# GabeTsai/YOLO-For-Turbines

Measured on AMD Instinct MI355X. Metric: images/sec at 416x416 (fwd), higher is better.
Workload: dtype f32; 1 GPU; BASELINE configs[1]: batch 32/GPU 416x416 fp32 inference, 80-class head, YOLOv3 forward (75 fused conv launches); per_gpu_batch=32, global_batch=32, image_size=416, num_classes=80, parallelism=image-sharded x1 (no collective)

## Files before the change

include/yolo_mi355x.h:

```cpp
#ifndef YOLO_MI355X_H
#define YOLO_MI355X_H

#include <stddef.h>
#include <stdint.h>

#ifdef __cplusplus
extern "C" {
#endif

#define YOLO_OK 0
#define YOLO_ERR_ARG (-1)
#define YOLO_ERR_UNSUPPORTED (-2)
#define YOLO_ERR_LAUNCH (-3)
#define YOLO_ERR_WORKSPACE (-4)

enum { YOLO_F32 = 0, YOLO_F16 = 1, YOLO_BF16 = 2 };
enum { YOLO_ACT_NONE = 0, YOLO_ACT_LEAKY = 1, YOLO_ACT_MISH = 2 };
enum { YOLO_OUT_NHWC = 0, YOLO_OUT_UPSAMPLE2X = 1, YOLO_OUT_HEAD = 2 };
enum { YOLO_FLAG_RESIDUAL = 1, YOLO_FLAG_NANCHECK = 2, YOLO_FLAG_FILTERS_READY = 4, YOLO_FLAG_SPLIT_BF16 = 8 };

typedef struct yolo_conv_desc {
    int32_t n, h, w;
    int32_t cin, cout;
    int32_t ksize, stride;
    int32_t x_ld, x_off;
    int32_t y_ld, y_off;
    int32_t r_ld, r_off;
    int32_t act;
    int32_t out_mode;
    int32_t dtype;
    int32_t flags;
    int32_t tile;
} yolo_conv_desc;

// ... 23 lines not shown
int yolo_stem_supported(int cin, int cout, int ksize, int stride);
int yolo_stem_pack(const float* w_oihw, float* w_k_major, int cout, void* stream);
int yolo_stem_fwd(const float* x_nchw, const float* w_k_major, const float* scale, const float* shift, void* y,
                  int n, int h, int w, int cout, int y_ld, int y_off, int act, int dtype, int32_t* nan_flag, void* stream);

int yolo_conv_fwd(const yolo_conv_desc* d, const void* x, const void* w_packed, const float* scale,
                  const float* shift, const void* residual, void* y, int32_t* nan_flag, void* stream);
int yolo_conv_fwd_batch(const yolo_conv_op* ops, int n_ops, int32_t* nan_flag, void* stream);
size_t yolo_conv_workspace_bytes(const yolo_conv_desc* d);
int yolo_conv_fwd_ws(const yolo_conv_desc* d, const void* x, const void* w_packed, const float* scale, const float* shift,
                     const void* residual, void* y, void* workspace, size_t workspace_bytes, int32_t* nan_flag, void* stream);
int yolo_conv_pick_tile(const yolo_conv_desc* d);
int yolo_conv_num_tiles(void);
int yolo_conv_split3_supported(const yolo_conv_desc* d);
int yolo_conv_split3_eligible(const yolo_conv_desc* d);
size_t yolo_wino4_filter_bytes(const yolo_conv_desc* d);
int yolo_wino4_filters(const yolo_conv_desc* d, const void* w_packed, void* U4, void* stream);
int yolo_conv_wino4_blocks(const yolo_conv_desc* d, int* whole, int* half);

size_t yolo_bn_workspace_bytes(int m, int c);
int yolo_bn_stats(const void* z, int m, int c, int ld, int off, const float* gamma, const float* beta, float momentum,
                  float eps, float* running_mean, float* running_var, float* mean, float* invstd, float* scale,
                  float* shift, int dtype, void* workspace, size_t workspace_bytes, void* stream);
int yolo_conv_stats_rows(const yolo_conv_desc* d, int* ld);
int yolo_conv_fwd_stats(const yolo_conv_desc* d, const void* x, const void* w_packed, void* z, float* stats, size_t stats_bytes,
                        void* stream);
int yolo_bn_stats_from_partials(const float* partial, int rows, int ld, int m, int c, const float* gamma, const float* beta,
                                float momentum, float eps, float* running_mean, float* running_var, float* mean, float* invstd,
                                float* scale, float* shift, void* stream);
int yolo_conv_bstats_rows(const yolo_conv_desc* d, int* ld);
// ... 127 lines not shown
```

yolo_for_turbines_amd/_lib.py:

```python
from __future__ import annotations

import ctypes as C
import os

_HERE = os.path.dirname(os.path.abspath(__file__))
LIB_PATH = os.environ.get("YOLO_MI355X_LIB") or os.path.join(_HERE, "libyolo_mi355x.so")

F32, F16, BF16 = 0, 1, 2
ACT_NONE, ACT_LEAKY, ACT_MISH = 0, 1, 2
OUT_NHWC, OUT_UPSAMPLE2X, OUT_HEAD = 0, 1, 2
FLAG_RESIDUAL, FLAG_NANCHECK, FLAG_FILTERS_READY, FLAG_SPLIT_BF16 = 1, 2, 4, 8


class PackItem(C.Structure):
    _fields_ = [("w_oihw", C.c_void_p), ("w_packed", C.c_void_p), ("cout", C.c_int), ("cin", C.c_int), ("ksize", C.c_int),
                ("reserved", C.c_int)]


class ConvDesc(C.Structure):
    _fields_ = [(n, C.c_int32) for n in (
        "n", "h", "w", "cin", "cout", "ksize", "stride", "x_ld", "x_off", "y_ld", "y_off", "r_ld", "r_off",
        "act", "out_mode", "dtype", "flags", "tile")]


class ConvOp(C.Structure):
    _fields_ = [("d", ConvDesc)] + [(n, C.c_uint64) for n in ("x", "w_packed", "scale", "shift", "residual", "y",
# ... 48 lines not shown
    "yolo_sgd_step_amp": (C.c_int, [C.c_void_p, C.c_int, C.c_void_p, C.c_int, C.c_void_p, C.c_void_p, C.c_void_p, C.c_void_p, C.c_int, C.c_int,
                                    C.c_void_p]),
    "yolo_stem_supported": (C.c_int, [C.c_int, C.c_int, C.c_int, C.c_int]),
    "yolo_stem_pack": (C.c_int, [C.c_void_p, C.c_void_p, C.c_int, C.c_void_p]),
    "yolo_stem_fwd": (C.c_int, [C.c_void_p, C.c_void_p, C.c_void_p, C.c_void_p, C.c_void_p, C.c_int, C.c_int, C.c_int,
                                C.c_int, C.c_int, C.c_int, C.c_int, C.c_int, C.c_void_p, C.c_void_p]),
    "yolo_conv_fwd": (C.c_int, [C.POINTER(ConvDesc), C.c_void_p, C.c_void_p, C.c_void_p, C.c_void_p, C.c_void_p,
                                C.c_void_p, C.c_void_p, C.c_void_p]),
    "yolo_conv_fwd_batch": (C.c_int, [C.POINTER(ConvOp), C.c_int, C.c_void_p, C.c_void_p]),
    "yolo_conv_workspace_bytes": (C.c_size_t, [C.POINTER(ConvDesc)]),
    "yolo_conv_fwd_ws": (C.c_int, [C.POINTER(ConvDesc), C.c_void_p, C.c_void_p, C.c_void_p, C.c_void_p, C.c_void_p,
                                   C.c_void_p, C.c_void_p, C.c_size_t, C.c_void_p, C.c_void_p]),
    "yolo_conv_pick_tile": (C.c_int, [C.POINTER(ConvDesc)]),
    "yolo_conv_split3_eligible": (C.c_int, [C.POINTER(ConvDesc)]),
    "yolo_conv_split3_supported": (C.c_int, [C.POINTER(ConvDesc)]),
    "yolo_conv_num_tiles": (C.c_int, []),
    "yolo_wino4_filter_bytes": (C.c_size_t, [C.POINTER(ConvDesc)]),
    "yolo_wino4_filters": (C.c_int, [C.POINTER(ConvDesc), C.c_void_p, C.c_void_p, C.c_void_p]),
    "yolo_conv_wino4_blocks": (C.c_int, [C.POINTER(ConvDesc), C.POINTER(C.c_int), C.POINTER(C.c_int)]),
    "yolo_bn_workspace_bytes": (C.c_size_t, [C.c_int, C.c_int]),
    "yolo_bn_stats": (C.c_int, [C.c_void_p, C.c_int, C.c_int, C.c_int, C.c_int, C.c_void_p, C.c_void_p, C.c_float, C.c_float,
                                C.c_void_p, C.c_void_p, C.c_void_p, C.c_void_p, C.c_void_p, C.c_void_p, C.c_int, C.c_void_p,
                                C.c_size_t, C.c_void_p]),
    "yolo_conv_stats_rows": (C.c_int, [C.POINTER(ConvDesc), C.POINTER(C.c_int)]),
    "yolo_conv_fwd_stats": (C.c_int, [C.POINTER(ConvDesc), C.c_void_p, C.c_void_p, C.c_void_p, C.c_void_p, C.c_size_t, C.c_void_p]),
    "yolo_bn_stats_from_partials": (C.c_int, [C.c_void_p, C.c_int, C.c_int, C.c_int, C.c_int, C.c_void_p, C.c_void_p, C.c_float, C.c_float,
                                              C.c_void_p, C.c_void_p, C.c_void_p, C.c_void_p, C.c_void_p, C.c_void_p, C.c_void_p]),
    "yolo_bn_act_fwd": (C.c_int, [C.c_void_p, C.c_int, C.c_int, C.c_void_p, C.c_void_p, C.c_void_p, C.c_void_p, C.c_int, C.c_int,
                                  C.c_void_p, C.c_int, C.c_int, C.c_int, C.c_int, C.c_int, C.c_int, C.c_int, C.c_int, C.c_int,
                                  C.c_void_p, C.c_void_p]),
# ... 108 lines not shown
```

yolo_for_turbines_amd/csrc/conv_f32.hip:

```cpp
#include "conv_f32_epilogue.h"

namespace yolo {

constexpr int LDS_LD = 36;


template <int BM, int BN, bool SMALLC>
__global__ __launch_bounds__(256) void conv_igemm_f32(const ConvArgs p) {
    constexpr int WM = BM / 2, WN = BN / 2;
    constexpr int TM = WM / 32, TN = WN / 32;
    constexpr int RA = BM / 32, RB = BN / 32;
    extern __shared__ __attribute__((aligned(16))) char smem_raw[];
    float* As = reinterpret_cast<float*>(smem_raw);
    float* Bs = As + 2 * BM * LDS_LD;

    const int tid = threadIdx.x;
    const int lane = tid & 63;
    const int wave = tid >> 6;
    const int wm = wave >> 1, wn = wave & 1;
    const int tile_n = blockIdx.x % p.tiles_n;
    const int tile_m = blockIdx.x / p.tiles_n;
    const int m0 = tile_m * BM, n0 = tile_n * BN;

    const int chunk = tid & 7;
// ... 165 lines not shown

static int conv_fwd_impl(const yolo_conv_desc* d, const void* x, const void* w, const float* scale, const float* shift,
                         const void* residual, void* y, void* ws, size_t ws_bytes, int32_t* nan_flag, hipStream_t s) {
    int rc = validate(d);
    if (rc) return rc;
    if (!x || !w || !scale || !shift || !y) return fail(YOLO_ERR_ARG, "conv: null pointer");
    if ((d->flags & YOLO_FLAG_RESIDUAL) && !residual) return fail(YOLO_ERR_ARG, "conv: residual flag without pointer");
    if ((d->flags & YOLO_FLAG_NANCHECK) && !nan_flag) return fail(YOLO_ERR_ARG, "conv: nancheck flag without pointer");
    const bool filters_ready = d->flags & YOLO_FLAG_FILTERS_READY;
    if (filters_ready && (d->dtype != YOLO_F32 || f32_family(d, residual, ws ? ws_bytes : 0) != F32Family::Wino4))
        return fail(YOLO_ERR_ARG, "conv: YOLO_FLAG_FILTERS_READY on a layer that does not run as Winograd F(4x4) (tile 15 with its workspace)");
    const bool split3 = d->flags & YOLO_FLAG_SPLIT_BF16;
    if (split3 && !split3_honoured(d, residual, ws ? ws_bytes : 0))
        return fail(YOLO_ERR_UNSUPPORTED, "conv: YOLO_FLAG_SPLIT_BF16 needs an fp32 layer of the direct kernels (no Winograd workspace in play) with "
                                          "ksize 1 or 3, stride 1 or 2 and cin %% 32 == 0");
    if (d->dtype != YOLO_F32) return conv_h16_launch(d, x, w, scale, shift, residual, y, nan_flag, s);
    ConvArgs a;
    a.x = (const float*)x; a.w = (const float*)w; a.scale = scale; a.shift = shift;
    a.res = (const float*)residual; a.y = (float*)y; a.nan_flag = nan_flag;
    a.N = d->n; a.H = d->h; a.W = d->w; a.Cin = cin_pad_of(d->cin); a.Cout = d->cout;
    a.ks = d->ksize; a.stride = d->stride; a.pad = d->ksize / 2;
    a.Ho = (d->h + 2 * a.pad - d->ksize) / d->stride + 1;
    a.Wo = (d->w + 2 * a.pad - d->ksize) / d->stride + 1;
    const long long M = (long long)d->n * a.Ho * a.Wo;
    if (M > 0x7fffffffLL) return fail(YOLO_ERR_UNSUPPORTED, "conv: N*Ho*Wo exceeds int32");
    a.M = (int)M;
    a.x_ld = d->x_ld; a.x_off = d->x_off; a.y_ld = d->y_ld; a.y_off = d->y_off; a.r_ld = d->r_ld; a.r_off = d->r_off;
    a.Kpad = kpad_of(d->cin, d->ksize);
    a.KT = a.Kpad / BK;
    a.act = d->act; a.out_mode = d->out_mode; a.flags = d->flags;
    a.nc5 = d->out_mode == YOLO_OUT_HEAD ? d->cout / 3 : 1;
    a.tiles_n = 0;
    const bool smallc = a.Cin == 4;
    if (split3) return conv_split3_launch(a, d->tile == kTileF32Rs ? 0 : d->tile, s);
    switch (f32_family(d, residual, ws ? ws_bytes : 0)) {
    case F32Family::Rs: return conv1_rs_launch(d, x, w, scale, shift, residual, y, nan_flag, s);
    case F32Family::Wino4:
        if (!wino4_supported(d)) return fail(YOLO_ERR_UNSUPPORTED, "conv: tile 15 needs fp32 3x3 stride 1 with NHWC output and channel counts %% 4 == 0");
        return conv_wino4_launch(d, x, filters_ready ? nullptr : (const float*)w, filters_ready ? (const float*)w : nullptr, scale, shift,
                                 residual, y, ws, ws_bytes, nan_flag, s);
    case F32Family::Wino: {
        if (!wino_supported(d)) return fail(YOLO_ERR_UNSUPPORTED, "conv: tile 13 needs fp32 3x3 stride 1 with NHWC output and channel counts %% 4 == 0");
        const float* U = (const float*)w + v0_packed_elems(d->cout, d->cin, d->ksize) + v2_frag_elems(d->cout, d->cin, d->ksize);
        return conv_wino_launch(d, x, U, scale, shift, residual, y, ws, ws_bytes, nan_flag, s);
    }
    case F32Family::Direct: break;
    }
    if (d->tile == kTileF32Rs) return fail(YOLO_ERR_UNSUPPORTED, "conv: tile 12 needs a 1x1 with 256 / 384 / 512 input channels and cout %% 128 == 0");
    const int t = d->tile ? d->tile : pick_direct_tile(d);
// ... 20 lines not shown
int yolo_conv_pick_tile(const yolo_conv_desc* d) {
    int rc = yolo::validate(d);
    if (rc) return rc;
    return yolo::pick_tile(d);
}

int yolo_conv_split3_supported(const yolo_conv_desc* d) {
    if (yolo::validate(d)) return 0;
    yolo_conv_desc h = *d;
    h.tile = 0;
    return yolo::split3_honoured(&h, nullptr, SIZE_MAX);
}

int yolo_conv_split3_eligible(const yolo_conv_desc* d) { return yolo_conv_split3_supported(d) && yolo::split3_eligible(d); }

int yolo_conv_fwd(const yolo_conv_desc* d, const void* x, const void* w_packed, const float* scale, const float* shift,
                  const void* residual, void* y, int32_t* nan_flag, void* stream) {
    return yolo::conv_fwd_impl(d, x, w_packed, scale, shift, residual, y, nullptr, 0, nan_flag, (hipStream_t)stream);
}

size_t yolo_conv_workspace_bytes(const yolo_conv_desc* d) {
    if (yolo::validate(d)) return 0;
    switch (yolo::f32_family(d, nullptr, SIZE_MAX)) {
    case yolo::F32Family::Wino4: return yolo::wino4_workspace_bytes(d);
    case yolo::F32Family::Wino: return yolo::wino_workspace_bytes(d);
    default: return 0;
    }
}

int yolo_conv_fwd_ws(const yolo_conv_desc* d, const void* x, const void* w_packed, const float* scale, const float* shift,
// ... 18 lines not shown
```

yolo_for_turbines_amd/csrc/conv_f32_epilogue.h:

```cpp
#pragma once
#include "common.h"

namespace yolo {

typedef float f32x16 __attribute__((ext_vector_type(16)));

struct ConvArgs {
    const float* x;
    const float* w;
    const float* scale;
    const float* shift;
    const float* res;
    float* y;
    int* nan_flag;
    int N, H, W, Cin, Cout, Ho, Wo, M;
    int ks, stride, pad;
    int x_ld, x_off, y_ld, y_off, r_ld, r_off;
    int Kpad, KT;
    int act, out_mode, flags;
    int nc5;
    int tiles_n;
};

constexpr int BK = 32;

bool split3_supported(const yolo_conv_desc* d);
bool split3_eligible(const yolo_conv_desc* d);
int conv_split3_launch(const ConvArgs& a, int tile, hipStream_t s);

template <int BM, int BN>
__device__ __forceinline__ void conv_f32_epilogue(const ConvArgs& p, f32x16 (&acc)[BM / 64][BN / 64], float* ost, int m0, int n0) {
    constexpr int WM = BM / 2, WN = BN / 2;
    constexpr int TM = WM / 32, TN = WN / 32;
    const int tid = threadIdx.x;
    const int lane = tid & 63;
    const int wave = tid >> 6;
    const int wm = wave >> 1, wn = wave & 1;
    const int frow = lane & 31, fh = lane >> 5;
    const int HoWo = p.Ho * p.Wo;
    const bool has_res = p.flags & YOLO_FLAG_RESIDUAL;
    const bool nan_chk = p.flags & YOLO_FLAG_NANCHECK;
    bool saw_nan = false;
    const bool aligned4 = ((p.y_ld | p.y_off) & 3) == 0 && (!has_res || ((p.r_ld | p.r_off) & 3) == 0);
// ... 93 lines not shown
```

yolo_for_turbines_amd/csrc/conv_split3_f32.hip:

```cpp
#include "conv_f32_epilogue.h"

namespace yolo {

typedef __bf16 s3_bf16x8 __attribute__((ext_vector_type(8)));
typedef unsigned int s3_u32x4 __attribute__((ext_vector_type(4)));

constexpr int S3_ROWB = 64;

__device__ __forceinline__ unsigned s3_pack(unsigned a, unsigned b) { return __builtin_amdgcn_perm(b, a, 0x07060302u); }

__device__ __forceinline__ void s3_split(const f32x4 v, u32x2& hi, u32x2& mid, u32x2& lo, f32x4& chk) {
    const s3_u32x4 vb = __builtin_bit_cast(s3_u32x4, v);
    const f32x4 h = __builtin_bit_cast(f32x4, vb & 0xffff0000u);
    const f32x4 r1 = v - h;
    const s3_u32x4 r1b = __builtin_bit_cast(s3_u32x4, r1);
    const f32x4 m = __builtin_bit_cast(f32x4, r1b & 0xffff0000u);
    const f32x4 r2 = r1 - m;
    const s3_u32x4 r2b = __builtin_bit_cast(s3_u32x4, r2);
    chk += r2 * 0.f;
    hi[0] = s3_pack(vb[0], vb[1]); hi[1] = s3_pack(vb[2], vb[3]);
    mid[0] = s3_pack(r1b[0], r1b[1]); mid[1] = s3_pack(r1b[2], r1b[3]);
    lo[0] = s3_pack(r2b[0], r2b[1]); lo[1] = s3_pack(r2b[2], r2b[3]);
}

template <int BM, int BN>
__global__ __launch_bounds__(256, 2) void conv_split3_f32(const ConvArgs p) {
    constexpr int WM = BM / 2, WN = BN / 2;
    constexpr int TM = WM / 32, TN = WN / 32;
    constexpr int RA = BM / 32, RB = BN / 32;
    constexpr bool DBUF = BM + BN <= 128;
    constexpr int A_BYTES = 3 * BM * S3_ROWB;
    constexpr int BUF_BYTES = 3 * (BM + BN) * S3_ROWB;
    extern __shared__ __attribute__((aligned(16))) char smem_raw[];

    const int tid = threadIdx.x;
    const int lane = tid & 63;
    const int wave = tid >> 6;
    const int wm = wave >> 1, wn = wave & 1;
    const int tile_n = blockIdx.x % p.tiles_n;
    const int tile_m = blockIdx.x / p.tiles_n;
    const int m0 = tile_m * BM, n0 = tile_n * BN;
    const int HoWo = p.Ho * p.Wo;

    auto row_geom = [&](int m, long long& base, unsigned& mask) {
        const bool mv = m < p.M;
        const int mm = mv ? m : 0;
        const int n = mm / HoWo;
// ... 5 lines not shown
        unsigned mk = 0;
        for (int kh = 0; kh < p.ks; ++kh)
            for (int kw = 0; kw < p.ks; ++kw)
                if (mv && (unsigned)(hi0 + kh) < (unsigned)p.H && (unsigned)(wi0 + kw) < (unsigned)p.W)
                    mk |= 1u << (kh * p.ks + kw);
        mask = mk;
    };

    const int chunk = tid & 7;
    const int lrow = tid >> 3;
    long long a_base[RA];
    unsigned a_mask[RA];
#pragma unroll
    for (int i = 0; i < RA; ++i) row_geom(m0 + lrow + 32 * i, a_base[i], a_mask[i]);
    const float* wrow = p.w + (size_t)(n0 + lrow) * p.Kpad + chunk * 4;

    f32x4 ra[RA], rb[RB];
    f32x4 chk = {0.f, 0.f, 0.f, 0.f};
    auto load_global = [&](int kt) {
        const int kg = kt * BK;
        const int tap = kg / p.Cin;
        const int coff = kg - tap * p.Cin + chunk * 4;
        const int kh = tap / p.ks, kw = tap - kh * p.ks;
        const long long toff = (long long)(kh * p.W + kw) * p.x_ld + coff;
#pragma unroll
        for (int i = 0; i < RA; ++i) {
            const bool v = (a_mask[i] >> tap) & 1u;
            f32x4 z = {0.f, 0.f, 0.f, 0.f};
            ra[i] = v ? *reinterpret_cast<const f32x4*>(p.x + a_base[i] + toff) : z;
        }
#pragma unroll
        for (int i = 0; i < RB; ++i)
            rb[i] = *reinterpret_cast<const f32x4*>(wrow + (size_t)(32 * i) * p.Kpad + kt * BK);
    };
    auto store_lds = [&](int buf) {
        char* a = smem_raw + buf * BUF_BYTES + lrow * S3_ROWB + (((chunk >> 1) ^ ((lrow >> 2) & 3)) * 16 + (chunk & 1) * 8);
        char* b = a + A_BYTES;
#pragma unroll
        for (int i = 0; i < RA; ++i) {
            u32x2 h, m, l;
            s3_split(ra[i], h, m, l, chk);
            *reinterpret_cast<u32x2*>(a + (0 * BM + 32 * i) * S3_ROWB) = h;
            *reinterpret_cast<u32x2*>(a + (1 * BM + 32 * i) * S3_ROWB) = m;
            *reinterpret_cast<u32x2*>(a + (2 * BM + 32 * i) * S3_ROWB) = l;
        }
#pragma unroll
        for (int i = 0; i < RB; ++i) {
            u32x2 h, m, l;
            s3_split(rb[i], h, m, l, chk);
            *reinterpret_cast<u32x2*>(b + (0 * BN + 32 * i) * S3_ROWB) = h;
            *reinterpret_cast<u32x2*>(b + (1 * BN + 32 * i) * S3_ROWB) = m;
            *reinterpret_cast<u32x2*>(b + (2 * BN + 32 * i) * S3_ROWB) = l;
        }
    };

    f32x16 acc[TM][TN];
#pragma unroll
    for (int i = 0; i < TM; ++i)
#pragma unroll
        for (int j = 0; j < TN; ++j)
#pragma unroll
            for (int r = 0; r < 16; ++r) acc[i][j][r] = 0.f;

    const int frow = lane & 31, fh = lane >> 5;
    const int a_frag = (wm * WM + frow) * S3_ROWB;
    const int b_frag = A_BYTES + (wn * WN + frow) * S3_ROWB;
    const int fsw = (frow >> 2) & 3;
    const int f_slot[2] = {(fh ^ fsw) * 16, ((2 + fh) ^ fsw) * 16};

    load_global(0);
    store_lds(0);
    __syncthreads();

    for (int kt = 0; kt < p.KT; ++kt) {
        const int cur = DBUF ? (kt & 1) : 0;
        const bool more = kt + 1 < p.KT;
        if (more) load_global(kt + 1);
        const char* Ab = smem_raw + cur * BUF_BYTES + a_frag;
        const char* Bb = smem_raw + cur * BUF_BYTES + b_frag;
#pragma unroll
        for (int c = 0; c < 2; ++c) {
            s3_bf16x8 af[TM][3], bf[TN][3];
#pragma unroll
            for (int i = 0; i < TM; ++i)
#pragma unroll
                for (int q = 0; q < 3; ++q)
                    af[i][q] = *reinterpret_cast<const s3_bf16x8*>(Ab + (q * BM + i * 32) * S3_ROWB + f_slot[c]);
#pragma unroll
            for (int j = 0; j < TN; ++j)
#pragma unroll
                for (int q = 0; q < 3; ++q)
                    bf[j][q] = *reinterpret_cast<const s3_bf16x8*>(Bb + (q * BN + j * 32) * S3_ROWB + f_slot[c]);
            constexpr int QA[6] = {0, 2, 1, 0, 1, 0};
            constexpr int QB[6] = {2, 0, 1, 1, 0, 0};
#pragma unroll
            for (int t = 0; t < 6; ++t)
#pragma unroll
                for (int i = 0; i < TM; ++i)
#pragma unroll
                    for (int j = 0; j < TN; ++j)
                        acc[i][j] = __builtin_amdgcn_mfma_f32_32x32x16_bf16(af[i][QA[t]], bf[j][QB[t]], acc[i][j], 0, 0, 0);
        }
        if (!DBUF) __syncthreads();
        if (more) store_lds(DBUF ? (cur ^ 1) : 0);
        __syncthreads();
    }

    const bool nonfinite = chk[0] != chk[0] || chk[1] != chk[1] || chk[2] != chk[2] || chk[3] != chk[3];
    if (__syncthreads_or(nonfinite)) {
        long long f_base[TM];
        unsigned f_mask[TM];
#pragma unroll
        for (int i = 0; i < TM; ++i) row_geom(m0 + wm * WM + i * 32 + frow, f_base[i], f_mask[i]);
        const float* fw = p.w + (size_t)(n0 + wn * WN + frow) * p.Kpad + 4 * fh;
#pragma unroll
        for (int i = 0; i < TM; ++i)
#pragma unroll
            for (int j = 0; j < TN; ++j)
#pragma unroll
                for (int r = 0; r < 16; ++r) acc[i][j][r] = 0.f;
        for (int kt = 0; kt < p.KT; ++kt) {
            const int kg = kt * BK;
            const int tap = kg / p.Cin;
// ... 14 lines not shown
                    for (int i = 0; i < TM; ++i)
#pragma unroll
                        for (int j = 0; j < TN; ++j)
                            acc[i][j] = __builtin_amdgcn_mfma_f32_32x32x2f32(af[i][e], bf[j][e], acc[i][j], 0, 0, 0);
            }
        }
    }

    conv_f32_epilogue<BM, BN>(p, acc, reinterpret_cast<float*>(smem_raw), m0, n0);
}

bool split3_supported(const yolo_conv_desc* d) {
    return d->dtype == YOLO_F32 && (d->ksize == 1 || d->ksize == 3) && (d->stride == 1 || d->stride == 2) && d->cin % 32 == 0;
}

template <int BM, int BN>
static int launch_split3(const ConvArgs& a, hipStream_t s) {
    constexpr size_t operands = (size_t)(BM + BN <= 128 ? 2 : 1) * 3 * (BM + BN) * S3_ROWB;
    constexpr size_t transpose = (size_t)BM * (BN + 4) * sizeof(float);
    constexpr size_t lds = operands > transpose ? operands : transpose;
    ConvArgs p = a;
    p.tiles_n = ceil_div(a.Cout, BN);
    const long long blocks = (long long)ceil_div(a.M, BM) * p.tiles_n;
    if (blocks > 0x7fffffffLL) return fail(YOLO_ERR_UNSUPPORTED, "conv_split3_f32: too many blocks");
    if (lds > 64 * 1024) {
        static LdsOnce once;
        if (int rc = reserve_lds(once, reinterpret_cast<const void*>(&conv_split3_f32<BM, BN>), lds, "conv_split3_f32")) return rc;
    }
    hipLaunchKernelGGL((conv_split3_f32<BM, BN>), dim3((unsigned)blocks), dim3(256), lds, s, p);
    return check_launch("conv_split3_f32");
}

static int pick_split3_tile(const ConvArgs& a) {
    if (a.ks == 3 && a.stride == 2 && a.Cin >= 64 && a.Cin < 512) return kTileF32Reg128x128;
    if (a.ks == 1 && (long long)a.H * a.W * a.Cout < 100000) return kTileF32Reg64x64;
    return kTileF32Reg128x64;
}

bool split3_eligible(const yolo_conv_desc* d) {
    if (!split3_supported(d)) return false;
    if (d->ksize == 3) return d->stride == 2 || (d->cin == 32 && (long long)d->h * d->w >= 208 * 208);
    return d->stride == 1 && (long long)d->h * d->w * d->cout >= 80000;
}

int conv_split3_launch(const ConvArgs& a, int tile, hipStream_t s) {
    switch (tile ? tile : pick_split3_tile(a)) {
    case kTileF32Reg128x128: return launch_split3<128, 128>(a, s);
    case kTileF32Reg128x64: return launch_split3<128, 64>(a, s);
    case kTileF32Reg64x64: return launch_split3<64, 64>(a, s);
    default: return fail(YOLO_ERR_UNSUPPORTED, "conv: YOLO_FLAG_SPLIT_BF16 has tiles 1 (128x128), 2 (128x64) and 4 (64x64), not %d", tile);
    }
}

}
```

yolo_for_turbines_amd/engine.py:

```python
from __future__ import annotations

import ctypes as C
import os
import weakref
from dataclasses import dataclass
from typing import Optional

import torch
import torch.nn as nn

from . import _lib as L

_DT = {"fp32": (L.F32, torch.float32), "fp16": (L.F16, torch.float16), "bf16": (L.BF16, torch.bfloat16)}


def resolve_dtype(requested=None):
    if requested is not None:
        if requested not in _DT:
            raise ValueError(f"compute dtype must be one of {sorted(_DT)}, got {requested!r}")
        return requested
    if torch.is_autocast_enabled():
        dt = torch.get_autocast_dtype("cuda")
        return "bf16" if dt == torch.bfloat16 else "fp16"
    return "fp32"
# ... 134 lines not shown
    return prog


class PackedBlock:

    def __init__(self, block, device, dtype="fp32"):
        cv = block.conv
        self.dtype = dtype
        self.code = _DT[dtype][0]
        lib = L.lib()
        stem_ok = bool(lib.yolo_stem_supported(cv.in_channels, cv.out_channels, cv.kernel_size[0], cv.stride[0]))
        n = lib.yolo_packed_weight_bytes(cv.out_channels, cv.in_channels, cv.kernel_size[0], self.code)
        if n == 0 and not (stem_ok and dtype != "fp32"):
            raise NotImplementedError(f"conv {cv.in_channels}->{cv.out_channels} k{cv.kernel_size[0]} has no {dtype} kernel "
                                      "(16-bit needs cin % 32 == 0)")
        self.w = torch.empty(max(n, 16), dtype=torch.uint8, device=device)
        self.scale = torch.empty(cv.out_channels, dtype=torch.float32, device=device)
        self.shift = torch.empty(cv.out_channels, dtype=torch.float32, device=device)
        self.stem_w = None
        self.packs_conv = n != 0
        if stem_ok:
            self.stem_w = torch.empty(27 * cv.out_channels, dtype=torch.float32, device=device)
        self.stamp = None
        self.u4 = None
        self.u4_desc = None
        self.u4_stamp = None
        self.fold_stamp = None
        self.folded = False

    @staticmethod
    def stamp_of(block):
        w, rest = PackedBlock.stamp_tensors(block)
        gen = block.__dict__.get("_pack_gen", 0)
        return ((w.data_ptr(), w._version, gen),), tuple((t.data_ptr(), t._version, gen) for t in rest)

    @staticmethod
    def stamp_tensors(block):
        mods = block._modules
        conv = mods["conv"]
        w = conv._parameters["weight"]
        if block.batch_norm_act:
# ... 14 lines not shown

    def want_u4(self, desc):
        if self.u4 is None:
            n = L.lib().yolo_wino4_filter_bytes(C.byref(desc))
            if n == 0:
                raise L.YoloLibError("yolo_wino4_filter_bytes: the layer cannot run as tile 15")
            self.u4_desc = L.ConvDesc.from_buffer_copy(desc)
            self.u4 = torch.empty(n, dtype=torch.uint8, device=self.w.device)
            self.u4_stamp = None
        return self.u4

    def refresh_u4(self, stream):
        L.check(L.lib().yolo_wino4_filters(C.byref(self.u4_desc), self.w.data_ptr(), self.u4.data_ptr(), stream), "yolo_wino4_filters")
        self.u4_stamp = self.stamp

    def refresh(self, block, stream, fold_bn=True, conv_packed=False, pack=True):
        lib = L.lib()
        cv = block.conv
        w = cv.weight.detach()
        if w.dtype != torch.float32 or not w.is_contiguous():
            w = w.float().contiguous()
        if pack:
            self.u4_stamp = None
            if self.packs_conv and not conv_packed:
                L.check(lib.yolo_pack_weights(w.data_ptr(), self.w.data_ptr(), cv.out_channels, cv.in_channels,
                                              cv.kernel_size[0], self.code, stream), "yolo_pack_weights")
            if self.stem_w is not None:
                L.check(lib.yolo_stem_pack(w.data_ptr(), self.stem_w.data_ptr(), cv.out_channels, stream), "yolo_stem_pack")
        self.folded = True
        if block.batch_norm_act and not fold_bn:
            self.folded = False
        elif block.batch_norm_act:
            bn = block.batch_norm
            g, b, m, v = (t.detach().float().contiguous() for t in (bn.weight, bn.bias, bn.running_mean, bn.running_var))
            L.check(lib.yolo_bn_fold(g.data_ptr(), b.data_ptr(), m.data_ptr(), v.data_ptr(), float(bn.eps),
                                     self.scale.data_ptr(), self.shift.data_ptr(), cv.out_channels, stream), "yolo_bn_fold")
        else:
            b = cv.bias.detach().float().contiguous()
# ... 74 lines not shown
            d.out_mode = op["out_mode"]
            d.dtype = self.code
            d.flags = op["flags"]
            d.tile = tile_override or 0
            if i >= self.first:
                e.x = self.phys[x.buf].data_ptr()
            e.w_packed, e.scale, e.shift = pk.w.data_ptr(), pk.scale.data_ptr(), pk.shift.data_ptr()
            if (dtype == "fp32" and i >= self.first and op["k"] == 3 and op["s"] == 1 and (tile_override or 0) in (0, 15)
                    and L.lib().yolo_conv_workspace_bytes(C.byref(d))
                    and (d.tile == 15 or L.lib().yolo_conv_pick_tile(C.byref(d)) == 15)):
                e.w_packed = pk.want_u4(d).data_ptr()
                d.flags |= L.FLAG_FILTERS_READY
            elif (dtype == "fp32" and state.split3 and i >= self.first and not tile_override
                    and (L.lib().yolo_conv_split3_supported if state.split3 == "all" else L.lib().yolo_conv_split3_eligible)(C.byref(d))):
                d.flags |= L.FLAG_SPLIT_BF16
            if i == 0 and self.stem is not None:
                self.stem_pk = pk
            if op["pred"] is not None:
                self.pred_ops[op["pred"]] = (i, op["Ho"], blk.conv.out_channels // 3)
        lib = L.lib()
        need = [lib.yolo_conv_workspace_bytes(C.byref(self.table[i].d)) if i >= self.first else 0 for i in range(n_ops)]
        self.workspace = torch.empty(max(need), dtype=torch.uint8, device=device) if n_ops and max(need) else None
        if self.workspace is not None:
            self.total_bytes += self.workspace.numel()
            for i, nb in enumerate(need):
                if nb:
                    self.table[i].workspace, self.table[i].workspace_bytes = self.workspace.data_ptr(), self.workspace.numel()
        self.blocks0 = self.blocks[:1]
        self.nan_flag = torch.zeros(1, dtype=torch.int32, device=device)
        self.dropped = False
# ... 64 lines not shown
        new.split3 = self.split3
        return new

    def head_dtype(self):
        if self.autocast_heads and torch.is_autocast_enabled():
            return torch.get_autocast_dtype("cuda")
        return torch.float32

    def invalidate(self, drop_plans=False):
        self._gen += 1
        self._fast.clear()
        for per_dev in self._packed.values():
            for pk in per_dev.values():
                pk.stamp = None
                pk.u4_stamp = None
                pk.fold_stamp = None
                pk.folded = False
        if drop_plans:
            self._packed = weakref.WeakKeyDictionary()
            for plan in self._plans.values():
                plan.dropped = True
            self._plans.clear()

    def packed(self, block, device, dtype="fp32"):
        per_dev = self._packed.get(block)
        if per_dev is None:
            per_dev = self._packed[block] = {}
        pk = per_dev.get((device.index, dtype))
        if pk is None:
            pk = per_dev[(device.index, dtype)] = PackedBlock(block, device, dtype)
# ... 40 lines not shown
                    items.append(L.PackItem(w.data_ptr(), pk.w.data_ptr(), cv.out_channels, cv.in_channels, cv.kernel_size[0], 0))
                    keep.append(id(pk))
            if items:
                arr = (L.PackItem * len(items))(*items)
                L.check(L.lib().yolo_pack_weights_batch(C.cast(arr, C.c_void_p), len(items), 0, _DT[dtype][0], stream), "yolo_pack_weights_batch")
                batched = set(keep)
        for blk, pk in stale:
            pk.refresh(blk, stream, fold_bn, conv_packed=id(pk) in batched)
        for blk, pk in refold:
            pk.refresh(blk, stream, True, pack=False)
        if fold_bn:
            for blk in blocks:
                pk = self.packed(blk, device, dtype)
                if pk.u4 is not None and (pk.u4_stamp is None or pk.u4_stamp != pk.stamp):
                    pk.refresh_u4(stream)

    def mark_unfolded(self, blocks):
        self._gen += 1
        for blk in blocks:
            per_dev = self._packed.get(blk)
            if per_dev:
                for pk in per_dev.values():
                    pk.folded = False
                    pk.fold_stamp = None

    def forward(self, model, x):
        if not isinstance(x, torch.Tensor) or x.dim() != 4:
            raise ValueError("expected a (B,C,H,W) tensor")
        if not x.is_cuda:
            raise RuntimeError("yolo_for_turbines_amd runs on MI355X only: move the model and the input to the GPU "
# ... 164 lines not shown
```

Measured before the change: 2644 images/s.

## Precompute bf16x3 split weight planes once and stream them via LDS-DMA

Adds a one-time preparation kernel that splits the packed fp32 weights into hi/mid/lo bf16 planes in the swizzled LDS layout, stored after the packed weights together with a per-32-row non-finite table. The split3 conv kernel can then copy the B operand straight into LDS (with global_load_lds DMA for some tiles) instead of reloading fp32 weights and splitting them again in every block at every k-step. Tile choice and the eligibility threshold are widened to use 128x128 tiles and split3 on more 1x1 layers. In exchange the weight buffers take more memory, LDS use grows for the DMA ring, and the preparation must be redone whenever the weights change.

Measured after the change: 2689 images/s, median of 6. 1.02x the previous value.

```diff
diff --git a/include/yolo_mi355x.h b/include/yolo_mi355x.h
--- a/include/yolo_mi355x.h
+++ b/include/yolo_mi355x.h
@@ -17,7 +17,8 @@
 enum { YOLO_F32 = 0, YOLO_F16 = 1, YOLO_BF16 = 2 };
 enum { YOLO_ACT_NONE = 0, YOLO_ACT_LEAKY = 1, YOLO_ACT_MISH = 2 };
 enum { YOLO_OUT_NHWC = 0, YOLO_OUT_UPSAMPLE2X = 1, YOLO_OUT_HEAD = 2 };
-enum { YOLO_FLAG_RESIDUAL = 1, YOLO_FLAG_NANCHECK = 2, YOLO_FLAG_FILTERS_READY = 4, YOLO_FLAG_SPLIT_BF16 = 8 };
+enum { YOLO_FLAG_RESIDUAL = 1, YOLO_FLAG_NANCHECK = 2, YOLO_FLAG_FILTERS_READY = 4, YOLO_FLAG_SPLIT_BF16 = 8,
+       YOLO_FLAG_SPLIT_WEIGHTS_READY = 16 };
 
 typedef struct yolo_conv_desc {
     int32_t n, h, w;
@@ -71,6 +72,8 @@
 int yolo_conv_num_tiles(void);
 int yolo_conv_split3_supported(const yolo_conv_desc* d);
 int yolo_conv_split3_eligible(const yolo_conv_desc* d);
+size_t yolo_split3_weight_bytes(const yolo_conv_desc* d);
+int yolo_split3_weights(const yolo_conv_desc* d, const void* w_packed, void* out, void* stream);
 size_t yolo_wino4_filter_bytes(const yolo_conv_desc* d);
 int yolo_wino4_filters(const yolo_conv_desc* d, const void* w_packed, void* U4, void* stream);
 int yolo_conv_wino4_blocks(const yolo_conv_desc* d, int* whole, int* half);
diff --git a/yolo_for_turbines_amd/_lib.py b/yolo_for_turbines_amd/_lib.py
--- a/yolo_for_turbines_amd/_lib.py
+++ b/yolo_for_turbines_amd/_lib.py
@@ -9,7 +9,7 @@
 F32, F16, BF16 = 0, 1, 2
 ACT_NONE, ACT_LEAKY, ACT_MISH = 0, 1, 2
 OUT_NHWC, OUT_UPSAMPLE2X, OUT_HEAD = 0, 1, 2
-FLAG_RESIDUAL, FLAG_NANCHECK, FLAG_FILTERS_READY, FLAG_SPLIT_BF16 = 1, 2, 4, 8
+FLAG_RESIDUAL, FLAG_NANCHECK, FLAG_FILTERS_READY, FLAG_SPLIT_BF16, FLAG_SPLIT_WEIGHTS_READY = 1, 2, 4, 8, 16
 
 
 class PackItem(C.Structure):
@@ -88,6 +88,8 @@
     "yolo_conv_pick_tile": (C.c_int, [C.POINTER(ConvDesc)]),
     "yolo_conv_split3_eligible": (C.c_int, [C.POINTER(ConvDesc)]),
     "yolo_conv_split3_supported": (C.c_int, [C.POINTER(ConvDesc)]),
+    "yolo_split3_weight_bytes": (C.c_size_t, [C.POINTER(ConvDesc)]),
+    "yolo_split3_weights": (C.c_int, [C.POINTER(ConvDesc), C.c_void_p, C.c_void_p, C.c_void_p]),
     "yolo_conv_num_tiles": (C.c_int, []),
     "yolo_wino4_filter_bytes": (C.c_size_t, [C.POINTER(ConvDesc)]),
     "yolo_wino4_filters": (C.c_int, [C.POINTER(ConvDesc), C.c_void_p, C.c_void_p, C.c_void_p]),
diff --git a/yolo_for_turbines_amd/csrc/conv_f32.hip b/yolo_for_turbines_amd/csrc/conv_f32.hip
--- a/yolo_for_turbines_amd/csrc/conv_f32.hip
+++ b/yolo_for_turbines_amd/csrc/conv_f32.hip
@@ -203,9 +203,11 @@
     if (split3 && !split3_honoured(d, residual, ws ? ws_bytes : 0))
         return fail(YOLO_ERR_UNSUPPORTED, "conv: YOLO_FLAG_SPLIT_BF16 needs an fp32 layer of the direct kernels (no Winograd workspace in play) with "
                                           "ksize 1 or 3, stride 1 or 2 and cin %% 32 == 0");
+    if ((d->flags & YOLO_FLAG_SPLIT_WEIGHTS_READY) && !split3)
+        return fail(YOLO_ERR_UNSUPPORTED, "conv: YOLO_FLAG_SPLIT_WEIGHTS_READY goes with YOLO_FLAG_SPLIT_BF16 only");
     if (d->dtype != YOLO_F32) return conv_h16_launch(d, x, w, scale, shift, residual, y, nan_flag, s);
     ConvArgs a;
-    a.x = (const float*)x; a.w = (const float*)w; a.scale = scale; a.shift = shift;
+    a.x = (const float*)x; a.w = (const float*)w; a.w_planes = nullptr; a.scale = scale; a.shift = shift;
     a.res = (const float*)residual; a.y = (float*)y; a.nan_flag = nan_flag;
     a.N = d->n; a.H = d->h; a.W = d->w; a.Cin = cin_pad_of(d->cin); a.Cout = d->cout;
     a.ks = d->ksize; a.stride = d->stride; a.pad = d->ksize / 2;
@@ -221,7 +223,10 @@
     a.nc5 = d->out_mode == YOLO_OUT_HEAD ? d->cout / 3 : 1;
     a.tiles_n = 0;
     const bool smallc = a.Cin == 4;
-    if (split3) return conv_split3_launch(a, d->tile == kTileF32Rs ? 0 : d->tile, s);
+    if (split3) {
+        if (d->flags & YOLO_FLAG_SPLIT_WEIGHTS_READY) a.w_planes = (const char*)w + split3_planes_offset(d);
+        return conv_split3_launch(a, d->tile == kTileF32Rs ? 0 : d->tile, s);
+    }
     switch (f32_family(d, residual, ws ? ws_bytes : 0)) {
     case F32Family::Rs: return conv1_rs_launch(d, x, w, scale, shift, residual, y, nan_flag, s);
     case F32Family::Wino4:
@@ -272,6 +277,15 @@
 
 int yolo_conv_split3_eligible(const yolo_conv_desc* d) { return yolo_conv_split3_supported(d) && yolo::split3_eligible(d); }
 
+size_t yolo_split3_weight_bytes(const yolo_conv_desc* d) { return d && yolo_conv_split3_supported(d) ? yolo::split3_weight_bytes(d) : 0; }
+
+int yolo_split3_weights(const yolo_conv_desc* d, const void* w_packed, void* out, void* stream) {
+    if (!d || !yolo_conv_split3_supported(d))
+        return yolo::fail(YOLO_ERR_UNSUPPORTED, "yolo_split3_weights: the library does not honour YOLO_FLAG_SPLIT_BF16 on this layer");
+    if (!w_packed || !out || ((uintptr_t)out & 15)) return yolo::fail(YOLO_ERR_ARG, "yolo_split3_weights: null or misaligned pointer");
+    return yolo::split3_weights_launch(d, w_packed, out, (hipStream_t)stream);
+}
+
 int yolo_conv_fwd(const yolo_conv_desc* d, const void* x, const void* w_packed, const float* scale, const float* shift,
                   const void* residual, void* y, int32_t* nan_flag, void* stream) {
     return yolo::conv_fwd_impl(d, x, w_packed, scale, shift, residual, y, nullptr, 0, nan_flag, (hipStream_t)stream);
diff --git a/yolo_for_turbines_amd/csrc/conv_f32_epilogue.h b/yolo_for_turbines_amd/csrc/conv_f32_epilogue.h
--- a/yolo_for_turbines_amd/csrc/conv_f32_epilogue.h
+++ b/yolo_for_turbines_amd/csrc/conv_f32_epilogue.h
@@ -8,6 +8,7 @@
 struct ConvArgs {
     const float* x;
     const float* w;
+    const char* w_planes;
     const float* scale;
     const float* shift;
     const float* res;
@@ -27,6 +28,9 @@
 bool split3_supported(const yolo_conv_desc* d);
 bool split3_eligible(const yolo_conv_desc* d);
 int conv_split3_launch(const ConvArgs& a, int tile, hipStream_t s);
+size_t split3_planes_offset(const yolo_conv_desc* d);
+size_t split3_weight_bytes(const yolo_conv_desc* d);
+int split3_weights_launch(const yolo_conv_desc* d, const void* w_packed, void* out, hipStream_t s);
 
 template <int BM, int BN>
 __device__ __forceinline__ void conv_f32_epilogue(const ConvArgs& p, f32x16 (&acc)[BM / 64][BN / 64], float* ost, int m0, int n0) {
diff --git a/yolo_for_turbines_amd/csrc/conv_split3_f32.hip b/yolo_for_turbines_amd/csrc/conv_split3_f32.hip
--- a/yolo_for_turbines_amd/csrc/conv_split3_f32.hip
+++ b/yolo_for_turbines_amd/csrc/conv_split3_f32.hip
@@ -6,6 +6,12 @@
 typedef unsigned int s3_u32x4 __attribute__((ext_vector_type(4)));
 
 constexpr int S3_ROWB = 64;
+
+__device__ __forceinline__ int s3_row_off(int r, int chunk) { return r * S3_ROWB + (((chunk >> 1) ^ ((r >> 2) & 3)) * 16 + (chunk & 1) * 8); }
+
+typedef const __attribute__((address_space(1))) void* s3_gptr;
+typedef __attribute__((address_space(3))) void* s3_lptr;
+__device__ __forceinline__ void s3_glds16(const void* g, void* l) { __builtin_amdgcn_global_load_lds((s3_gptr)g, (s3_lptr)l, 16, 0, 0); }
 
 __device__ __forceinline__ unsigned s3_pack(unsigned a, unsigned b) { return __builtin_amdgcn_perm(b, a, 0x07060302u); }
 
@@ -23,14 +29,47 @@
     lo[0] = s3_pack(r2b[0], r2b[1]); lo[1] = s3_pack(r2b[2], r2b[3]);
 }
 
-template <int BM, int BN>
+struct S3PrepArgs {
+    const float* w;
+    char* out;
+    int Kpad, KT, cp;
+};
+
+__global__ __launch_bounds__(256) void split3_weights_f32(const S3PrepArgs p) {
+    const int tid = threadIdx.x;
+    const int chunk = tid & 7;
+    const int n = blockIdx.x * 32 + (tid >> 3);
+    const size_t plane_b = (size_t)p.cp * S3_ROWB;
+    const float* src = p.w + (size_t)n * p.Kpad + chunk * 4;
+    char* dst = p.out + s3_row_off(n, chunk);
+    f32x4 chk = {0.f, 0.f, 0.f, 0.f};
+    for (int kt = 0; kt < p.KT; ++kt) {
+        const f32x4 v = *reinterpret_cast<const f32x4*>(src + kt * BK);
+        u32x2 h, m, l;
+        s3_split(v, h, m, l, chk);
+        char* d = dst + (size_t)kt * 3 * plane_b;
+        *reinterpret_cast<u32x2*>(d) = h;
+        *reinterpret_cast<u32x2*>(d + plane_b) = m;
+        *reinterpret_cast<u32x2*>(d + 2 * plane_b) = l;
+    }
+    const bool nonfinite = chk[0] != chk[0] || chk[1] != chk[1] || chk[2] != chk[2] || chk[3] != chk[3];
+    const int any = __syncthreads_or(nonfinite);
+    if (tid == 0) reinterpret_cast<unsigned*>(p.out + (size_t)p.KT * 3 * plane_b)[blockIdx.x] = any ? 1u : 0u;
+}
+
+template <int BM, int BN, bool WREADY, bool WDMA>
 __global__ __launch_bounds__(256, 2) void conv_split3_f32(const ConvArgs p) {
+    static_assert(WREADY || !WDMA, "LDS-DMA needs the prepared weights");
     constexpr int WM = BM / 2, WN = BN / 2;
     constexpr int TM = WM / 32, TN = WN / 32;
     constexpr int RA = BM / 32, RB = BN / 32;
     constexpr bool DBUF = BM + BN <= 128;
     constexpr int A_BYTES = 3 * BM * S3_ROWB;
-    constexpr int BUF_BYTES = 3 * (BM + BN) * S3_ROWB;
+    constexpr int B_BYTES = 3 * BN * S3_ROWB;
+    constexpr int BUF_BYTES = A_BYTES + B_BYTES;
+    constexpr bool BRING = DBUF || WDMA;
+    constexpr int B_SLOT = DBUF ? BUF_BYTES : B_BYTES;
+    constexpr int PB = BN / 64;
     extern __shared__ __attribute__((aligned(16))) char smem_raw[];
 
     const int tid = threadIdx.x;
@@ -66,8 +105,12 @@
 #pragma unroll
     for (int i = 0; i < RA; ++i) row_geom(m0 + lrow + 32 * i, a_base[i], a_mask[i]);
     const float* wrow = p.w + (size_t)(n0 + lrow) * p.Kpad + chunk * 4;
+    const char* wq = p.w_planes;
+    const size_t plane_b = (size_t)((p.Cout + 127) & ~127) * S3_ROWB;
+    const char* wsrc = wq + (size_t)n0 * S3_ROWB + tid * 16;
 
     f32x4 ra[RA], rb[RB];
+    s3_u32x4 rw[3][PB];
     f32x4 chk = {0.f, 0.f, 0.f, 0.f};
     auto load_global = [&](int kt) {
         const int kg = kt * BK;
@@ -81,13 +124,27 @@
             f32x4 z = {0.f, 0.f, 0.f, 0.f};
             ra[i] = v ? *reinterpret_cast<const f32x4*>(p.x + a_base[i] + toff) : z;
         }
-#pragma unroll
-        for (int i = 0; i < RB; ++i)
-            rb[i] = *reinterpret_cast<const f32x4*>(wrow + (size_t)(32 * i) * p.Kpad + kt * BK);
+        if constexpr (!WREADY) {
+#pragma unroll
+            for (int i = 0; i < RB; ++i)
+                rb[i] = *reinterpret_cast<const f32x4*>(wrow + (size_t)(32 * i) * p.Kpad + kt * BK);
+        } else {
+            const char* src = wsrc + (size_t)kt * 3 * plane_b;
+            char* dst = smem_raw + A_BYTES + (kt & 1) * B_SLOT + wave * 1024;
+#pragma unroll
+            for (int q = 0; q < 3; ++q)
+#pragma unroll
+                for (int i = 0; i < PB; ++i) {
+                    if constexpr (WDMA)
+                        s3_glds16(src + q * plane_b + i * 4096, dst + q * BN * S3_ROWB + i * 4096);
+                    else
+                        rw[q][i] = *reinterpret_cast<const s3_u32x4*>(src + q * plane_b + i * 4096);
+                }
+        }
     };
-    auto store_lds = [&](int buf) {
-        char* a = smem_raw + buf * BUF_BYTES + lrow * S3_ROWB + (((chunk >> 1) ^ ((lrow >> 2) & 3)) * 16 + (chunk & 1) * 8);
-        char* b = a + A_BYTES;
+    auto store_lds = [&](int buf, int bslot) {
+        char* a = smem_raw + buf * BUF_BYTES + s3_row_off(lrow, chunk);
+        char* b = smem_raw + A_BYTES + bslot * B_SLOT + s3_row_off(lrow, chunk);
 #pragma unroll
         for (int i = 0; i < RA; ++i) {
             u32x2 h, m, l;
@@ -96,13 +153,21 @@
             *reinterpret_cast<u32x2*>(a + (1 * BM + 32 * i) * S3_ROWB) = m;
             *reinterpret_cast<u32x2*>(a + (2 * BM + 32 * i) * S3_ROWB) = l;
         }
-#pragma unroll
-        for (int i = 0; i < RB; ++i) {
-            u32x2 h, m, l;
-            s3_split(rb[i], h, m, l, chk);
-            *reinterpret_cast<u32x2*>(b + (0 * BN + 32 * i) * S3_ROWB) = h;
-            *reinterpret_cast<u32x2*>(b + (1 * BN + 32 * i) * S3_ROWB) = m;
-            *reinterpret_cast<u32x2*>(b + (2 * BN + 32 * i) * S3_ROWB) = l;
+        if constexpr (!WREADY) {
+#pragma unroll
+            for (int i = 0; i < RB; ++i) {
+                u32x2 h, m, l;
+                s3_split(rb[i], h, m, l, chk);
+                *reinterpret_cast<u32x2*>(b + (0 * BN + 32 * i) * S3_ROWB) = h;
+                *reinterpret_cast<u32x2*>(b + (1 * BN + 32 * i) * S3_ROWB) = m;
+                *reinterpret_cast<u32x2*>(b + (2 * BN + 32 * i) * S3_ROWB) = l;
+            }
+        } else if constexpr (!WDMA) {
+            char* bw = smem_raw + A_BYTES + bslot * B_SLOT + tid * 16;
+#pragma unroll
+            for (int q = 0; q < 3; ++q)
+#pragma unroll
+                for (int i = 0; i < PB; ++i) *reinterpret_cast<s3_u32x4*>(bw + q * BN * S3_ROWB + i * 4096) = rw[q][i];
         }
     };
 
@@ -121,15 +186,17 @@
     const int f_slot[2] = {(fh ^ fsw) * 16, ((2 + fh) ^ fsw) * 16};
 
     load_global(0);
-    store_lds(0);
+    store_lds(0, 0);
+    if constexpr (WDMA) asm volatile("s_waitcnt vmcnt(0)" ::: "memory");
     __syncthreads();
 
     for (int kt = 0; kt < p.KT; ++kt) {
         const int cur = DBUF ? (kt & 1) : 0;
+        const int bcur = BRING ? (kt & 1) : 0;
         const bool more = kt + 1 < p.KT;
         if (more) load_global(kt + 1);
         const char* Ab = smem_raw + cur * BUF_BYTES + a_frag;
-        const char* Bb = smem_raw + cur * BUF_BYTES + b_frag;
+        const char* Bb = smem_raw + bcur * B_SLOT + b_frag;
 #pragma unroll
         for (int c = 0; c < 2; ++c) {
             s3_bf16x8 af[TM][3], bf[TN][3];
@@ -154,11 +221,17 @@
                         acc[i][j] = __builtin_amdgcn_mfma_f32_32x32x16_bf16(af[i][QA[t]], bf[j][QB[t]], acc[i][j], 0, 0, 0);
         }
         if (!DBUF) __syncthreads();
-        if (more) store_lds(DBUF ? (cur ^ 1) : 0);
+        if (more) store_lds(DBUF ? (cur ^ 1) : 0, BRING ? (bcur ^ 1) : 0);
+        if constexpr (WDMA) asm volatile("s_waitcnt vmcnt(0)" ::: "memory");
         __syncthreads();
     }
 
-    const bool nonfinite = chk[0] != chk[0] || chk[1] != chk[1] || chk[2] != chk[2] || chk[3] != chk[3];
+    bool nonfinite = chk[0] != chk[0] || chk[1] != chk[1] || chk[2] != chk[2] || chk[3] != chk[3];
+    if constexpr (WREADY) {
+        const unsigned* table = reinterpret_cast<const unsigned*>(wq + (size_t)p.KT * 3 * plane_b);
+#pragma unroll
+        for (int g = 0; g < BN / 32; ++g) nonfinite |= table[n0 / 32 + g] != 0;
+    }
     if (__syncthreads_or(nonfinite)) {
         long long f_base[TM];
         unsigned f_mask[TM];
@@ -203,9 +276,10 @@
     return d->dtype == YOLO_F32 && (d->ksize == 1 || d->ksize == 3) && (d->stride == 1 || d->stride == 2) && d->cin % 32 == 0;
 }
 
-template <int BM, int BN>
+template <int BM, int BN, bool WREADY, bool WDMA>
 static int launch_split3(const ConvArgs& a, hipStream_t s) {
-    constexpr size_t operands = (size_t)(BM + BN <= 128 ? 2 : 1) * 3 * (BM + BN) * S3_ROWB;
+    constexpr bool dbuf = BM + BN <= 128;
+    constexpr size_t operands = dbuf ? (size_t)2 * 3 * (BM + BN) * S3_ROWB : (size_t)3 * (BM + (WDMA ? 2 : 1) * BN) * S3_ROWB;
     constexpr size_t transpose = (size_t)BM * (BN + 4) * sizeof(float);
     constexpr size_t lds = operands > transpose ? operands : transpose;
     ConvArgs p = a;
@@ -214,29 +288,63 @@
     if (blocks > 0x7fffffffLL) return fail(YOLO_ERR_UNSUPPORTED, "conv_split3_f32: too many blocks");
     if (lds > 64 * 1024) {
         static LdsOnce once;
-        if (int rc = reserve_lds(once, reinterpret_cast<const void*>(&conv_split3_f32<BM, BN>), lds, "conv_split3_f32")) return rc;
-    }
-    hipLaunchKernelGGL((conv_split3_f32<BM, BN>), dim3((unsigned)blocks), dim3(256), lds, s, p);
+        if (int rc = reserve_lds(once, reinterpret_cast<const void*>(&conv_split3_f32<BM, BN, WREADY, WDMA>), lds, "conv_split3_f32")) return rc;
+    }
+    hipLaunchKernelGGL((conv_split3_f32<BM, BN, WREADY, WDMA>), dim3((unsigned)blocks), dim3(256), lds, s, p);
     return check_launch("conv_split3_f32");
 }
 
-static int pick_split3_tile(const ConvArgs& a) {
-    if (a.ks == 3 && a.stride == 2 && a.Cin >= 64 && a.Cin < 512) return kTileF32Reg128x128;
+constexpr bool kS3Dma128x128 = true, kS3Dma128x64 = false, kS3Dma64x64 = true;
+
+template <int BM, int BN, bool WDMA>
+static int launch_split3(const ConvArgs& a, hipStream_t s) {
+    return a.w_planes ? launch_split3<BM, BN, true, WDMA>(a, s) : launch_split3<BM, BN, false, false>(a, s);
+}
+
+size_t split3_planes_offset(const yolo_conv_desc* d) {
+    return (yolo_packed_weight_bytes(d->cout, d->cin, d->ksize, YOLO_F32) + 15) & ~(size_t)15;
+}
+
+size_t split3_weight_bytes(const yolo_conv_desc* d) {
+    const size_t cp = coutpad_of(d->cout), KT = kpad_of(d->cin, d->ksize) / BK;
+    return split3_planes_offset(d) + KT * 3 * cp * S3_ROWB + cp / 32 * sizeof(unsigned);
+}
+
+int split3_weights_launch(const yolo_conv_desc* d, const void* w_packed, void* out, hipStream_t s) {
+    const size_t off = split3_planes_offset(d);
+    if (out != w_packed) {
+        const char *a = static_cast<const char*>(w_packed), *b = static_cast<const char*>(out);
+        if (a < b + split3_weight_bytes(d) && b < a + off) return fail(YOLO_ERR_ARG, "yolo_split3_weights: out overlaps w_packed (pass the same pointer to prepare in place)");
+        if (hipMemcpyAsync(out, w_packed, off, hipMemcpyDeviceToDevice, s) != hipSuccess) return check_launch("yolo_split3_weights: copy");
+    }
+    S3PrepArgs p;
+    p.w = static_cast<const float*>(w_packed);
+    p.out = static_cast<char*>(out) + off;
+    p.Kpad = kpad_of(d->cin, d->ksize);
+    p.KT = p.Kpad / BK;
+    p.cp = coutpad_of(d->cout);
+    hipLaunchKernelGGL(split3_weights_f32, dim3(p.cp / 32), dim3(256), 0, s, p);
+    return check_launch("split3_weights_f32");
+}
+
+static int pick_split3_tile(const ConvArgs& a, bool ready) {
+    if (a.ks == 3 && a.stride == 2 && a.Cin >= 64 && (ready || a.Cin < 512)) return kTileF32Reg128x128;
     if (a.ks == 1 && (long long)a.H * a.W * a.Cout < 100000) return kTileF32Reg64x64;
+    if (ready && a.ks == 1 && a.Cout % 128 == 0 && a.Cin >= ((long long)a.H * a.W >= 52 * 52 ? 256 : 768)) return kTileF32Reg128x128;
     return kTileF32Reg128x64;
 }
 
 bool split3_eligible(const yolo_conv_desc* d) {
     if (!split3_supported(d)) return false;
     if (d->ksize == 3) return d->stride == 2 || (d->cin == 32 && (long long)d->h * d->w >= 208 * 208);
-    return d->stride == 1 && (long long)d->h * d->w * d->cout >= 80000;
+    return d->stride == 1 && (long long)d->h * d->w * d->cout >= 40000;
 }
 
 int conv_split3_launch(const ConvArgs& a, int tile, hipStream_t s) {
-    switch (tile ? tile : pick_split3_tile(a)) {
-    case kTileF32Reg128x128: return launch_split3<128, 128>(a, s);
-    case kTileF32Reg128x64: return launch_split3<128, 64>(a, s);
-    case kTileF32Reg64x64: return launch_split3<64, 64>(a, s);
+    switch (tile ? tile : pick_split3_tile(a, a.w_planes != nullptr)) {
+    case kTileF32Reg128x128: return launch_split3<128, 128, kS3Dma128x128>(a, s);
+    case kTileF32Reg128x64: return launch_split3<128, 64, kS3Dma128x64>(a, s);
+    case kTileF32Reg64x64: return launch_split3<64, 64, kS3Dma64x64>(a, s);
     default: return fail(YOLO_ERR_UNSUPPORTED, "conv: YOLO_FLAG_SPLIT_BF16 has tiles 1 (128x128), 2 (128x64) and 4 (64x64), not %d", tile);
     }
 }
diff --git a/yolo_for_turbines_amd/engine.py b/yolo_for_turbines_amd/engine.py
--- a/yolo_for_turbines_amd/engine.py
+++ b/yolo_for_turbines_amd/engine.py
@@ -172,7 +172,12 @@
         if n == 0 and not (stem_ok and dtype != "fp32"):
             raise NotImplementedError(f"conv {cv.in_channels}->{cv.out_channels} k{cv.kernel_size[0]} has no {dtype} kernel "
                                       "(16-bit needs cin % 32 == 0)")
-        self.w = torch.empty(max(n, 16), dtype=torch.uint8, device=device)
+        room = 0
+        if dtype == "fp32" and n and (cv.kernel_size[0] == 1 or cv.stride[0] == 2 or min(cv.in_channels, cv.out_channels) < 64):
+            d = L.ConvDesc(n=1, h=8, w=8, cin=cv.in_channels, cout=cv.out_channels, ksize=cv.kernel_size[0], stride=cv.stride[0],
+                           x_ld=(cv.in_channels + 3) // 4 * 4, y_ld=cv.out_channels, dtype=self.code)
+            room = lib.yolo_split3_weight_bytes(C.byref(d))
+        self.w = torch.empty(max(n, room, 16), dtype=torch.uint8, device=device)
         self.scale = torch.empty(cv.out_channels, dtype=torch.float32, device=device)
         self.shift = torch.empty(cv.out_channels, dtype=torch.float32, device=device)
         self.stem_w = None
@@ -183,6 +188,9 @@
         self.u4 = None
         self.u4_desc = None
         self.u4_stamp = None
+        self.s3 = None
+        self.s3_desc = None
+        self.s3_stamp = None
         self.fold_stamp = None
         self.folded = False
 
@@ -227,6 +235,20 @@
         L.check(L.lib().yolo_wino4_filters(C.byref(self.u4_desc), self.w.data_ptr(), self.u4.data_ptr(), stream), "yolo_wino4_filters")
         self.u4_stamp = self.stamp
 
+    def want_s3(self, desc):
+        if self.s3 is None:
+            n = L.lib().yolo_split3_weight_bytes(C.byref(desc))
+            if n == 0 or n > self.w.numel():
+                return None
+            self.s3_desc = L.ConvDesc.from_buffer_copy(desc)
+            self.s3 = self.w[:n]
+            self.s3_stamp = None
+        return self.s3
+
+    def refresh_s3(self, stream):
+        L.check(L.lib().yolo_split3_weights(C.byref(self.s3_desc), self.w.data_ptr(), self.w.data_ptr(), stream), "yolo_split3_weights")
+        self.s3_stamp = self.stamp
+
     def refresh(self, block, stream, fold_bn=True, conv_packed=False, pack=True):
         lib = L.lib()
         cv = block.conv
@@ -235,6 +257,7 @@
             w = w.float().contiguous()
         if pack:
             self.u4_stamp = None
+            self.s3_stamp = None
             if self.packs_conv and not conv_packed:
                 L.check(lib.yolo_pack_weights(w.data_ptr(), self.w.data_ptr(), cv.out_channels, cv.in_channels,
                                               cv.kernel_size[0], self.code, stream), "yolo_pack_weights")
@@ -339,6 +362,8 @@
             elif (dtype == "fp32" and state.split3 and i >= self.first and not tile_override
                     and (L.lib().yolo_conv_split3_supported if state.split3 == "all" else L.lib().yolo_conv_split3_eligible)(C.byref(d))):
                 d.flags |= L.FLAG_SPLIT_BF16
+                if state.split3 != "inflight" and pk.want_s3(d) is not None:
+                    d.flags |= L.FLAG_SPLIT_WEIGHTS_READY
             if i == 0 and self.stem is not None:
                 self.stem_pk = pk
             if op["pred"] is not None:
@@ -433,6 +458,7 @@
             for pk in per_dev.values():
                 pk.stamp = None
                 pk.u4_stamp = None
+                pk.s3_stamp = None
                 pk.fold_stamp = None
                 pk.folded = False
         if drop_plans:
@@ -503,6 +529,8 @@
                 pk = self.packed(blk, device, dtype)
                 if pk.u4 is not None and (pk.u4_stamp is None or pk.u4_stamp != pk.stamp):
                     pk.refresh_u4(stream)
+                if pk.s3 is not None and (pk.s3_stamp is None or pk.s3_stamp != pk.stamp):
+                    pk.refresh_s3(stream)
 
     def mark_unfolded(self, blocks):
         self._gen += 1
```
